# zerohd4869/MM-DFN

Measured on AMD Instinct MI355X. Metric: utterances/sec (fwd+bwd), IEMOCAP-shaped batch, higher is better.
Workload: dtype f32; 1 GPU; cfg2 (BASELINE configs[1]): B=16 dialogues/GPU, L=110, dims 100/100/512, 2 GCN layers, P=2, dropout 0.50; utterances_per_gpu=1760, parallelism=dp1

## Files before the change

### mm_dfn_amd/build.py

```python
import hashlib
import os
import shutil
import subprocess
import sys

HERE = os.path.dirname(os.path.abspath(__file__))
CSRC = os.path.join(HERE, "csrc")
LIBDIR = os.path.join(HERE, "lib")
LIBPATH = os.path.join(LIBDIR, "libmmdfn_hip.so")
TUNING_LIBPATH = os.path.join(LIBDIR, "libmmdfn_hip_tuning.so")
INCLUDE = os.path.join(os.path.dirname(HERE), "include")
ARCH = "gfx950"
NO_SPILL = {"gru.hip": ("gru_seq_bwd_kpart_kernelILi8ELi4ELi0ELi1E", "gru_seq_bwd_riders_kernelILb1E",
                        "gru_seq_fwd_io_kernelILi0ELi0ELi0ELi1E", "gru_seq_fwd_io_flags_kernelILi1E"),
            "lstm_seq.hip": ("lstm_seq_fwd_kernel", "lstm_seq_bwd_kernel"),
            "dialogue_rnn.hip": ("drnn_seq_fwd_kernel", "drnn_seq_bwd_kernel"),
            "cnn_features.hip": ("cnn_pool_fwd_kernel",)}


def sources():
    return sorted(os.path.join(CSRC, f) for f in os.listdir(CSRC) if f.endswith(".hip"))


def _digest():
    h = hashlib.sha256()
    files = sources() + sorted(os.path.join(CSRC, f) for f in os.listdir(CSRC) if f.endswith(".h"))
    files.append(os.path.join(INCLUDE, "mmdfn_hip.h"))
    for f in files:
        h.update(f.encode())
        with open(f, "rb") as fh:
            h.update(fh.read())
    return h.hexdigest()


def hipcc():
    exe = shutil.which("hipcc") or "/opt/rocm/bin/hipcc"
    if not os.path.exists(exe):
        raise RuntimeError("hipcc not found; libmmdfn_hip.so cannot be built")
    return exe


def build(force=False, verbose=True, tuning=False):
    import fcntl
    os.makedirs(LIBDIR, exist_ok=True)
    with open(os.path.join(LIBDIR, ".build.lock"), "w") as lock:
        fcntl.flock(lock, fcntl.LOCK_EX)
        try:
            return _build_locked(force, verbose, tuning)
        finally:
            fcntl.flock(lock, fcntl.LOCK_UN)


def _paths(tuning):
    lib = TUNING_LIBPATH if tuning else LIBPATH
    return lib, lib[:-3] + ".sha256", ("tuning_" if tuning else "")


def _build_locked(force, verbose, tuning):
    lib, stamp, prefix = _paths(tuning)
    digest = _digest()
    if not force and os.path.exists(lib) and os.path.exists(stamp):
        with open(stamp) as fh:
            if fh.read().strip() == digest:
                return lib
    objs = []
    jobs = []
    for src in sources():
        obj = os.path.join(LIBDIR, prefix + os.path.basename(src)[:-4] + ".o")
        cmd = [hipcc(), "--offload-arch=" + ARCH, "-O3", "-std=c++17", "-fPIC", "-I", INCLUDE, "-c", src, "-o", obj]
        if tuning:
            cmd.insert(1, "-DMMDFN_TUNING")
        if verbose:
            print(" ".join(cmd), flush=True)
        watch = NO_SPILL.get(os.path.basename(src))
        if watch:
            cmd.append("-Rpass-analysis=kernel-resource-usage")
            jobs.append((cmd, subprocess.Popen(cmd, stderr=subprocess.PIPE, text=True), watch))
        else:
            jobs.append((cmd, subprocess.Popen(cmd), None))
        objs.append(obj)
    for cmd, proc, watch in jobs:
        err = proc.communicate()[1] if watch else None
        if proc.wait() != 0:
            if err:
                sys.stderr.write(err)
            raise subprocess.CalledProcessError(proc.returncode, cmd)
        if watch:
            _check_no_spill(err, watch, cmd)
    cmd = [hipcc(), "--offload-arch=" + ARCH, "-shared", "-fPIC", "-o", lib] + objs
    if verbose:
        print(" ".join(cmd), flush=True)
    subprocess.check_call(cmd)
    with open(stamp, "w") as fh:
        fh.write(digest)
    return lib


def _check_no_spill(remarks, watch, cmd):
    name = None
    seen = set()
    for line in remarks.splitlines():
        if "Function Name:" in line:
            name = line.split("Function Name:")[1].split()[0]
        elif "ScratchSize [bytes/lane]:" in line and name and any(w in name for w in watch):
            seen.update(w for w in watch if w in name)
            if int(line.split("ScratchSize [bytes/lane]:")[1].split()[0]) != 0:
                raise RuntimeError("%s spills registers (%s): build.NO_SPILL lists it as a kernel that must run without "
                                   "scratch traffic" % (name, line.strip()))
    if len(seen) != len(watch):
        raise RuntimeError("no resource-usage remark for kernels matching %r (%s)" % (sorted(set(watch) - seen), " ".join(cmd)))


def is_stale(tuning=False):
    lib, stamp, _ = _paths(tuning)
    if not (os.path.exists(lib) and os.path.exists(stamp)):
        return True
    with open(stamp) as fh:
        return fh.read().strip() != _digest()


if __name__ == "__main__":
    print(build(force="--force" in sys.argv, tuning="--tuning" in sys.argv))
```

### mm_dfn_amd/csrc/gru.hip

```cpp
#include "mmdfn_internal.h"
#include "gemm_tn_split_body.h"
#include <type_traits>
#include <utility>
#include "keep_flags_body.h"
#include "../../include/mmdfn_hip.h"
#include <stdlib.h>

namespace {

constexpr int GH = 100;
constexpr int NT = 256;
constexpr int MAXG = 4;

constexpr int SCHED_MAX = 2048;
constexpr int MAXSEG = 16;

struct SegInfo {
    const int32_t* rank[MAXG];
    int P[MAXG];
    int BP[MAXG];
    int tdir[MAXG];
    int nslot;
    int slot_g[2 * MAXG];
    int slot_d[2 * MAXG];
// ... 1219 lines not shown
    };
    auto stash_block = [&](int buf) {
#pragma unroll
        for (int e = 0; e < NIN; ++e) {
            const int idx = tid + e * NTK;
            if (idx < TB * IN4) *reinterpret_cast<float4*>(&in_s[buf][0][0] + 4 * idx) = stage[e];
        }
    };
    auto flush_block = [&](int b) {
        for (int idx = tid; idx < TB * OUT4; idx += NTK) {
            const int sl = idx / OUT4;
            const int c4 = idx - sl * OUT4;
            const int sidx = b * TB + sl;
            if (sidx >= T) continue;
            int t;
            const int rw = step_row(sidx, t);
            const float4 v = *reinterpret_cast<const float4*>(&out_s[sl][4 * c4]);
            const int64_t o = ((int64_t)t * rows + rw) * (6 * GH) + dir * 3 * GH;
            if (c4 < 3 * GH / 4)
                *reinterpret_cast<float4*>(dgi + o + 4 * c4) = v;
            else
                __builtin_nontemporal_store(__builtin_bit_cast(f32x4, v), reinterpret_cast<f32x4*>(dgh + o + 4 * (c4 - 3 * GH / 4)));
        }
    };

    load_block(0);
    stash_block(0);
    if (nblocks > 1) load_block(1);
    __syncthreads();

    auto seg_end = [&](int prow) {
        if (dhinit != nullptr && ch.trunc) {
            f32x2 acc0 = {0.f, 0.f}, acc1 = {0.f, 0.f};
#pragma unroll
            for (int jj = 0; jj < JPW; ++jj) {
                const float dj = lane_bcast(dv[jj / 64], jj % 64);
                const f32x2 dd = {dj, dj};
                if (jj & 1) acc1 = __builtin_elementwise_fma(w[jj], dd, acc1);
                else acc0 = __builtin_elementwise_fma(w[jj], dd, acc0);
            }
            constexpr int PX = SEG ? 2 : 0;
            part[PX][wv][lane] = acc0[0] + acc1[0];
            part[PX][wv][lane + 64] = acc0[1] + acc1[1];
            __syncthreads();
#pragma unroll
            for (int q = 0; q < NGR; ++q) {
                float pr[NW];
#pragma unroll
                for (int w2 = 0; w2 < NW; ++w2) pr[w2] = part[PX][w2][uu[q]];
#pragma unroll
                for (int sp = 1; sp < NW; sp *= 2)
#pragma unroll
                    for (int w2 = 0; w2 + sp < NW; w2 += 2 * sp) pr[w2] += pr[w2 + sp];
                if (has[q] && gg[q] == 0) dhinit[(int64_t)prow * GH + uu[q]] = carry[q] + pr[0];
            }
        }
#pragma unroll
        for (int q = 0; q < NGR; ++q) {
            dv[q] = 0.f;
            carry[q] = 0.f;
        }
    };

    int step = 0;
    int seg_p = 0, bnd = 0x7fffffff;
    if constexpr (SEG) {
        int q = ch.nseg - 1;
        while (q >= 0 && seg_k[q] == 0) --q;
        int q2 = q - 1;
        while (q2 >= 0 && seg_k[q2] == 0) --q2;
        seg_p = __builtin_amdgcn_readfirstlane(q < 0 ? 0 : q);
        bnd = __builtin_amdgcn_readfirstlane(q2 >= 0 ? seg_k[q] : 0x7fffffff);
    }
    for (int b = 0; b < nblocks; ++b) {
        const int buf = b & 1;
        for (int sl = 0; sl < TB && step < T; ++sl, ++step) {
            const int pb = step & 1;
            if constexpr (SEG) {
                if (step == bnd) {
                    seg_end(row + seg_p);
                    int q = seg_p - 1;
                    while (q >= 0 && seg_k[q] == 0) --q;
                    seg_p = __builtin_amdgcn_readfirstlane(q);
                    int q2 = q - 1;
                    while (q2 >= 0 && seg_k[q2] == 0) --q2;
                    bnd = __builtin_amdgcn_readfirstlane(q2 >= 0 ? bnd + seg_k[q] : 0x7fffffff);
                }
            }
            const float* ip = &in_s[buf][sl][0];
            float iv[NGR][6];
#pragma unroll
            for (int q = 0; q < NGR; ++q)
#pragma unroll
                for (int e = 0; e < 6; ++e) iv[q][e] = ip[e * GH + uu[q]];
            f32x2 acc0 = {0.f, 0.f}, acc1 = {0.f, 0.f};
#pragma unroll
            for (int j4 = 0; j4 < JPW; j4 += GRP) {
                float dj[GRP];
#pragma unroll
                for (int e = 0; e < GRP; ++e) dj[e] = (j4 + e < JPW) ? lane_bcast(dv[(j4 + e) / 64], (j4 + e) % 64) : 0.f;
                if (GRP == 4) asm volatile("" : "+s"(dj[0]), "+s"(dj[GRP > 1 ? 1 : 0]), "+s"(dj[GRP > 2 ? 2 : 0]), "+s"(dj[GRP > 3 ? 3 : 0]));
#pragma unroll
                for (int e = 0; e < GRP; ++e) {
                    if (j4 + e >= JPW) continue;
                    const f32x2 dd = {dj[e], dj[e]};
                    if ((j4 + e) & 1) acc1 = __builtin_elementwise_fma(w[j4 + e], dd, acc1);
                    else acc0 = __builtin_elementwise_fma(w[j4 + e], dd, acc0);
                }
            }
            part[pb][wv][lane] = acc0[0] + acc1[0];
            part[pb][wv][lane + 64] = acc0[1] + acc1[1];
            __syncthreads();
            float* orow = &out_s[sl][0];
#pragma unroll
            for (int q = 0; q < NGR; ++q) {
                const int un = uu[q];
                float pr[NW];
#pragma unroll
                for (int w2 = 0; w2 < NW; ++w2) pr[w2] = part[pb][w2][un];
#pragma unroll
                for (int sp = 1; sp < NW; sp *= 2)
#pragma unroll
                    for (int w2 = 0; w2 + sp < NW; w2 += 2 * sp) pr[w2] += pr[w2 + sp];
                const float rec = pr[0];
                const float dh = iv[q][0] + carry[q] + rec;
                const float rr = iv[q][1], zz = iv[q][2], nn = iv[q][3], ghn = iv[q][4], hprev = iv[q][5];
                const float dn = dh * (1.0f - zz);
                const float dz = dh * (hprev - nn);
                carry[q] = dh * zz;
                const float dnpre = dn * (1.0f - nn * nn);
                const float drpre = dnpre * ghn * rr * (1.0f - rr);
                const float dzpre = dz * zz * (1.0f - zz);
                const float dghn = dnpre * rr;
                const float gi_v = gg[q] == 0 ? drpre : (gg[q] == 1 ? dzpre : dnpre);
                const float gh_v = gg[q] == 0 ? drpre : (gg[q] == 1 ? dzpre : dghn);
                if (has[q]) {
                    orow[jr[q]] = gi_v;
                    orow[3 * GH + jr[q]] = gh_v;
                }
                dv[q] = gh_v;
            }
        }
        __syncthreads();
        if (b + 1 < nblocks) stash_block(buf ^ 1);
        flush_block(b);
        if (b + 2 < nblocks) load_block(b + 2);
        __syncthreads();
    }
    if constexpr (SEG) {
        if (T > 0) seg_end(row + seg_p);
    }
}

constexpr int BWD_RING_D = 4;
constexpr int BWD_DIRECT_PART_B = 2 * 8 * PU * (int)sizeof(float);
constexpr int BWD_DIRECT_LDS = 84 * 1024;

static_assert(GH == 100, "the plane offsets of the direct body's requests are literals: 400 / 800 / 1200 bytes");
#define GRU_VM_LOAD(dst, off, base, lit) \
    asm volatile("global_load_dword %0, %1, %2" lit : "+v"(dst) : "v"(off), "s"(base))
template <int N>
__device__ __forceinline__ void vm_wait6(float (&r)[6]) {
    asm volatile("s_waitcnt vmcnt(%6)" : "+v"(r[0]), "+v"(r[1]), "+v"(r[2]), "+v"(r[3]), "+v"(r[4]), "+v"(r[5]) : "n"(N));
}

__device__ __forceinline__ void vm_store2(uint32_t off, float gi_v, float* pi, float gh_v, float* ph) {
    asm volatile("global_store_dword %0, %1, %2" : : "v"(off), "v"(gi_v), "s"(pi) : "memory");
    asm volatile("global_store_dword %0, %1, %2 nt" : : "v"(off), "v"(gh_v), "s"(ph) : "memory");
}
template <class F, int... K>
__device__ __forceinline__ void static_for(F& f, std::integer_sequence<int, K...>) {
    (f(std::integral_constant<int, K>{}), ...);
}
template <int J, int N, class F>
__device__ __forceinline__ void static_while(F& f, const int rem) {
    if constexpr (J < N) {
        if (J < rem) {
            f(std::integral_constant<int, J>{});
            static_while<J + 1, N>(f, rem);
        }
    }
}

__device__ __forceinline__ void gru_bwd_direct_body(const BwdGroups& G, const int bx, const int by, unsigned char* dyn) {
    constexpr int NW = 8, GRP = 4;
    constexpr int JPW = (3 * GH + NW - 1) / NW;
    constexpr int D = BWD_RING_D, NS = D + 1;
    static_assert(JPW <= 64, "a lane owns one gate row");
    static_assert(D >= 1 && D <= 7, "s_waitcnt vmcnt(8 D) must fit the 6-bit immediate");
    float (*part)[NW][PU] = reinterpret_cast<float (*)[NW][PU]>(dyn);

    int gidx = 0;
    while (gidx + 1 < G.n && bx >= G.slice0[gidx + 1]) ++gidx;
    const int dir = by;
    const int row = bx - G.slice0[gidx];
    const int T = G.T[gidx];
    const int rows = G.rows[gidx];
    if (T <= 0) return;
    const int tid = threadIdx.x, lane = tid & 63, wv = tid >> 6;
    const int j0 = JPW * wv;
    const float* __restrict__ dy = G.dy[gidx];
    const float* __restrict__ y = G.y[gidx];
    const float* __restrict__ gates = G.gates[gidx];
    const float* __restrict__ w_hh = G.w_hh[2 * gidx + dir];
    float* __restrict__ dgi = G.dgi[gidx];
    float* __restrict__ dgh = G.dgh[gidx];
    static_assert(3 * GH - (NW - 1) * JPW > 0, "every wave owns a gate row");

    const bool has1 = lane + 64 < GH;
    f32x2 w[JPW];
#pragma unroll
    for (int jj = 0; jj < JPW; ++jj) {
        const bool jok = j0 + jj < 3 * GH;
        const int jc = jok ? j0 + jj : 3 * GH - 1;
        w[jj][0] = jok ? w_hh[(int64_t)jc * GH + lane] : 0.f;
        w[jj][1] = (jok && has1) ? w_hh[(int64_t)jc * GH + lane + 64] : 0.f;
    }
#pragma unroll
    for (int jj = 0; jj < JPW; ++jj) pin_loaded(w[jj]);
    const bool has = lane < JPW && j0 + lane < 3 * GH;
    const int jr = has ? j0 + lane : 0;
    const int gg = jr / GH;
    const int uu = jr - gg * GH;
    uint32_t uoff = (uint32_t)uu * 4u, joff = (uint32_t)jr * 4u;
    float dv = 0.f, carry = 0.f;

    const int64_t dt = dir ? 1 : -1;
    const int64_t o0 = (int64_t)(dir ? 0 : T - 1) * rows + row;
    const int64_t st_y = dt * rows * (2 * GH), st_g = dt * rows * (8 * GH), st_o = dt * rows * (6 * GH);
    const float* pd = dy + o0 * (2 * GH) + dir * GH;
    const float* pg = gates + (o0 * 2 + dir) * (4 * GH);
    const float* py = y + o0 * (2 * GH) + dir * GH + (T > 1 ? st_y : 0);
    float* pi = dgi + o0 * (6 * GH) + dir * 3 * GH;
    float* ph = dgh + o0 * (6 * GH) + dir * 3 * GH;
    int f = 0;
    auto fetch = [&](float (&o6)[6]) {
        GRU_VM_LOAD(o6[0], uoff, pd, "");
        GRU_VM_LOAD(o6[1], uoff, pg, "");
        GRU_VM_LOAD(o6[2], uoff, pg, " offset:400");
        GRU_VM_LOAD(o6[3], uoff, pg, " offset:800");
        GRU_VM_LOAD(o6[4], uoff, pg, " offset:1200");
        GRU_VM_LOAD(o6[5], uoff, py, "");
        pd += (f + 1 < T) ? st_y : 0;
        pg += (f + 1 < T) ? st_g : 0;
        py += (f + 2 < T) ? st_y : 0;
        ++f;
    };

    float ring[NS][6];
#pragma unroll
    for (int k = 0; k < NS; ++k)
#pragma unroll
        for (int e = 0; e < 6; ++e) ring[k][e] = 0.f;
#pragma unroll
    for (int k = 0; k < D; ++k) fetch(ring[k]);

    auto run_step = [&](auto NC, const int step, float (&iv)[6]) {
        const int pb = step & 1;
        f32x2 acc0 = {0.f, 0.f}, acc1 = {0.f, 0.f};
#pragma unroll
        for (int j4 = 0; j4 < JPW; j4 += GRP) {
            float dj[GRP];
#pragma unroll
            for (int e = 0; e < GRP; ++e) dj[e] = (j4 + e < JPW) ? lane_bcast(dv, j4 + e) : 0.f;
            asm volatile("" : "+s"(dj[0]), "+s"(dj[1]), "+s"(dj[2]), "+s"(dj[3]));
#pragma unroll
            for (int e = 0; e < GRP; ++e) {
                if (j4 + e >= JPW) continue;
                const f32x2 dd = {dj[e], dj[e]};
                if ((j4 + e) & 1) acc1 = __builtin_elementwise_fma(w[j4 + e], dd, acc1);
                else acc0 = __builtin_elementwise_fma(w[j4 + e], dd, acc0);
            }
        }
        part[pb][wv][lane] = acc0[0] + acc1[0];
        part[pb][wv][lane + 64] = acc0[1] + acc1[1];
        __syncthreads();
        float pr[NW];
#pragma unroll
        for (int w2 = 0; w2 < NW; ++w2) pr[w2] = part[pb][w2][uu];
#pragma unroll
        for (int sp = 1; sp < NW; sp *= 2)
#pragma unroll
            for (int w2 = 0; w2 + sp < NW; w2 += 2 * sp) pr[w2] += pr[w2 + sp];
        const float rec = pr[0];
        vm_wait6<decltype(NC)::value>(iv);
        const float dh = iv[0] + carry + rec;
        const float rr = iv[1], zz = iv[2], nn = iv[3], ghn = iv[4];
        const float hprev = (step < T - 1) ? iv[5] : 0.f;
        const float dn = dh * (1.0f - zz);
        const float dz = dh * (hprev - nn);
        carry = dh * zz;
        float nn2 = nn * nn;
        asm("" : "+v"(nn2));
        const float dnpre = dn * (1.0f - nn2);
        const float drpre = dnpre * ghn * rr * (1.0f - rr);
        const float dzpre = dz * zz * (1.0f - zz);
        const float dghn = dnpre * rr;
        const float gi_v = gg == 0 ? drpre : (gg == 1 ? dzpre : dnpre);
        const float gh_v = gg == 0 ? drpre : (gg == 1 ? dzpre : dghn);
        dv = gh_v;
        asm volatile("" : "+v"(carry), "+v"(dv));
        if (has) {
            vm_store2(joff, gi_v, pi, gh_v, ph);
        }
        pi += st_o;
        ph += st_o;
    };

    const int T_trips = T - T % NS;
    for (int s0 = 0; s0 < T_trips; s0 += NS) {
        auto trip_step = [&](auto K) {
            constexpr int k = decltype(K)::value;
            fetch(ring[(k + D) % NS]);
            run_step(std::integral_constant<int, (6 * D + 2 * k < 8 * D ? 6 * D + 2 * k : 8 * D)>{}, s0 + k, ring[k]);
        };
        static_for(trip_step, std::make_integer_sequence<int, NS>{});
    }
    auto tail_step = [&](auto J) {
        constexpr int j = decltype(J)::value;
        run_step(std::integral_constant<int, 6 * (D - 1 - j) + 2 * j>{}, T_trips + j, ring[j]);
    };
    static_while<0, D>(tail_step, T - T_trips);
}

#ifndef MMDFN_FWD_RING_D
#define MMDFN_FWD_RING_D BWD_RING_D
#endif
#ifndef MMDFN_FWD_PAIR_STORES
#define MMDFN_FWD_PAIR_STORES 1
#endif
constexpr int FWD_RING_D = MMDFN_FWD_RING_D;
constexpr int FWD_PAIR_STORES = MMDFN_FWD_PAIR_STORES;
constexpr int FWD_DIRECT_LDS = BWD_DIRECT_LDS;

template <int N>
__device__ __forceinline__ void vm_wait3(float (&r)[3]) {
    asm volatile("s_waitcnt vmcnt(%3)" : "+v"(r[0]), "+v"(r[1]), "+v"(r[2]) : "n"(N));
}
#define GRU_VM_STORE(off, val, base, lit) \
    asm volatile("global_store_dword %0, %1, %2" lit : : "v"(off), "v"(val), "s"(base) : "memory")

__device__ __forceinline__ void gru_fwd_direct_body(const FwdGroups& G, const int bx, const int by) {
    constexpr int D = FWD_RING_D, NS = D + 1;
    constexpr int L = 3, S = FWD_PAIR_STORES ? 3 : 5;
    static_assert(D >= 1 && (L + S) * D <= 63, "s_waitcnt vmcnt((L + S) D) must fit the 6-bit immediate");
    __shared__ __attribute__((aligned(16))) float hs[2][GH + 4];

    int gidx = 0;
    while (gidx + 1 < G.n && bx >= G.slice0[gidx + 1]) ++gidx;
    const int dir = by;
    const int row = bx - G.slice0[gidx];
    const int T = G.T[gidx];
    const int rows = G.rows[gidx];
    if (T <= 0) return;
    const int tid = threadIdx.x;
    const int u = tid >> 1;
    const int half = tid & 1;
    const bool active = u < GH;
    const int uu = active ? u : GH - 1;
    const int kbase = half ? KH0 : 0;
    const int klen = half ? GH - KH0 : KH0;
    const float* __restrict__ gi = G.gi[gidx];
    const float* __restrict__ w_hh = G.w_hh[2 * gidx + dir];
    const float* __restrict__ b_hh = G.b_hh[2 * gidx + dir];
    float* __restrict__ y = G.y[gidx];
    float* __restrict__ gates = G.gates[gidx];
    f32x2 wr[KW / 2], wz[KW / 2], wn[KW / 2];
#pragma unroll
    for (int k = 0; k < KW; ++k) {
        const bool ok = k < klen;
        const int kk = kbase + (ok ? k : 0);
        wr[k >> 1][k & 1] = ok ? w_hh[(int64_t)(0 * GH + uu) * GH + kk] : 0.f;
        wz[k >> 1][k & 1] = ok ? w_hh[(int64_t)(1 * GH + uu) * GH + kk] : 0.f;
        wn[k >> 1][k & 1] = ok ? w_hh[(int64_t)(2 * GH + uu) * GH + kk] : 0.f;
    }
#pragma unroll
    for (int k = 0; k < KW / 2; ++k) {
        pin_loaded(wr[k]);
        pin_loaded(wz[k]);
        pin_loaded(wn[k]);
    }
    float bhr = b_hh[uu], bhz = b_hh[GH + uu], bhn = b_hh[2 * GH + uu];
    pin_loaded(bhr);
    pin_loaded(bhz);
    pin_loaded(bhn);
    const bool mine = active && half == 0;
    float hprev = 0.f;
    for (int i = tid; i < 2 * (GH + 4); i += NT) (&hs[0][0])[i] = 0.f;
    __syncthreads();

    const int64_t dt = dir ? -1 : 1;
    const int64_t o0 = (int64_t)(dir ? T - 1 : 0) * rows + row;
    const int64_t st_i = dt * rows * (6 * GH), st_y = dt * rows * (2 * GH), st_g = dt * rows * (8 * GH);
    const float* pi = gi + o0 * (6 * GH) + dir * 3 * GH;
    float* py = y + o0 * (2 * GH) + dir * GH;
    float* pg = gates + (o0 * 2 + dir) * (4 * GH);
    uint32_t ioff = (uint32_t)uu * 4u;
    uint32_t yoff = (uint32_t)uu * 4u;
    uint32_t goff = (uint32_t)uu * 4u + (FWD_PAIR_STORES && half ? 4u * GH : 0u);
    asm volatile("" : "+v"(ioff), "+v"(yoff), "+v"(goff));
    int f = 0;
    auto fetch = [&](float (&o3)[3]) {
        GRU_VM_LOAD(o3[0], ioff, pi, "");
        GRU_VM_LOAD(o3[1], ioff, pi, " offset:400");
        GRU_VM_LOAD(o3[2], ioff, pi, " offset:800");
        pi += (f + 1 < T) ? st_i : 0;
        ++f;
    };

    float ring[NS][3];
#pragma unroll
    for (int k = 0; k < NS; ++k)
#pragma unroll
        for (int e = 0; e < 3; ++e) ring[k][e] = 0.f;
#pragma unroll
    for (int k = 0; k < D; ++k) fetch(ring[k]);

    auto run_step = [&](auto NC, auto REQ, const int step, float (&iv)[3], float (&nx)[3]) {
        const int cur = step & 1;
        f32x2 ar0 = {0.f, 0.f}, az0 = {0.f, 0.f}, an0 = {0.f, 0.f}, ar1 = {0.f, 0.f}, az1 = {0.f, 0.f}, an1 = {0.f, 0.f};
        constexpr int HLOOK = 6;
        const uint32_t haddr = (uint32_t)(uintptr_t)((__attribute__((address_space(3))) const float*)(&hs[cur][kbase]));
        f32x4 hb[HLOOK];
#define GRU_LDS_RD(J)                                                                                        \
    asm volatile("ds_read_b128 %0, %1 offset:%2" : "=&v"(hb[(J) % HLOOK]) : "v"(haddr), "i"(16 * (J)) : "memory")
#define GRU_LDS_WAIT(N, J) asm volatile("s_waitcnt lgkmcnt(" #N ")" : "+v"(hb[(J) % HLOOK]) : : "memory")
#define GRU_GROUP(K4)                                                                                        \
    do {                                                                                                     \
        const f32x4 h4 = hb[(K4) % HLOOK];                                                                   \
        const f32x2 ha = {h4.x, h4.y}, hb2 = {h4.z, h4.w};                                                   \
        ar0 = __builtin_elementwise_fma(wr[2 * (K4)], ha, ar0);                                              \
        az0 = __builtin_elementwise_fma(wz[2 * (K4)], ha, az0);                                              \
        an0 = __builtin_elementwise_fma(wn[2 * (K4)], ha, an0);                                              \
        ar1 = __builtin_elementwise_fma(wr[2 * (K4) + 1], hb2, ar1);                                         \
        az1 = __builtin_elementwise_fma(wz[2 * (K4) + 1], hb2, az1);                                         \
        an1 = __builtin_elementwise_fma(wn[2 * (K4) + 1], hb2, an1);                                         \
    } while (0)
        GRU_LDS_RD(0); GRU_LDS_RD(1); GRU_LDS_RD(2); GRU_LDS_RD(3); GRU_LDS_RD(4); GRU_LDS_RD(5);
        if constexpr (decltype(REQ)::value) fetch(nx);
        GRU_LDS_WAIT(5, 0); GRU_GROUP(0); GRU_LDS_RD(6);
        GRU_LDS_WAIT(5, 1); GRU_GROUP(1); GRU_LDS_RD(7);
        GRU_LDS_WAIT(5, 2); GRU_GROUP(2); GRU_LDS_RD(8);
        GRU_LDS_WAIT(5, 3); GRU_GROUP(3); GRU_LDS_RD(9);
        GRU_LDS_WAIT(5, 4); GRU_GROUP(4); GRU_LDS_RD(10);
        GRU_LDS_WAIT(5, 5); GRU_GROUP(5); GRU_LDS_RD(11);
        GRU_LDS_WAIT(5, 6); GRU_GROUP(6); GRU_LDS_RD(12);
        GRU_LDS_WAIT(5, 7); GRU_GROUP(7);
        GRU_LDS_WAIT(4, 8); GRU_GROUP(8);
        GRU_LDS_WAIT(3, 9); GRU_GROUP(9);
        GRU_LDS_WAIT(2, 10); GRU_GROUP(10);
        GRU_LDS_WAIT(1, 11); GRU_GROUP(11);
        GRU_LDS_WAIT(0, 12); GRU_GROUP(12);
#undef GRU_GROUP
#undef GRU_LDS_WAIT
#undef GRU_LDS_RD
        float ar = (ar0.x + ar0.y) + (ar1.x + ar1.y);
        float az = (az0.x + az0.y) + (az1.x + az1.y);
        float an = (an0.x + an0.y) + (an1.x + an1.y);
        ar += pair_swap(ar);
        az += pair_swap(az);
        an += pair_swap(an);
        vm_wait3<decltype(NC)::value>(iv);
        const float g0 = iv[0], g1 = iv[1], g2 = iv[2];
        float ghn = an + bhn;
        float rr = sigmoidf_(g0 + ar + bhr);
        float zz = sigmoidf_(g1 + az + bhz);
        float nn = tanhf_(g2 + rr * ghn);
        float hnew = (1.0f - zz) * nn + zz * hprev;
        if (mine) hs[cur ^ 1][u] = hnew;
        asm volatile("" : "+v"(hnew), "+v"(rr), "+v"(zz), "+v"(nn), "+v"(ghn));
        hprev = hnew;
        if constexpr (FWD_PAIR_STORES) {
            const float va = half ? zz : rr, vb = half ? ghn : nn;
            if (active) {
                GRU_VM_STORE(goff, va, pg, " nt");
                GRU_VM_STORE(goff, vb, pg, " offset:800 nt");
                if (mine) GRU_VM_STORE(yoff, hnew, py, "");
            }
        } else {
            if (mine) {
                GRU_VM_STORE(yoff, hnew, py, "");
                GRU_VM_STORE(goff, rr, pg, " nt");
                GRU_VM_STORE(goff, zz, pg, " offset:400 nt");
                GRU_VM_STORE(goff, nn, pg, " offset:800 nt");
                GRU_VM_STORE(goff, ghn, pg, " offset:1200 nt");
            }
        }
        py += st_y;
        pg += st_g;
        __syncthreads();
    };

    const int T_trips = T - T % NS;
    const std::true_type yes{};
    const std::false_type no{};
    if (T_trips > 0) {
        auto first_step = [&](auto K) {
            constexpr int k = decltype(K)::value;
            run_step(std::integral_constant<int, L * D + S * k>{}, yes, k, ring[k], ring[(k + D) % NS]);
        };
        static_for(first_step, std::make_integer_sequence<int, NS>{});
        for (int s0 = NS; s0 < T_trips; s0 += NS) {
            auto trip_step = [&](auto K) {
                constexpr int k = decltype(K)::value;
                run_step(std::integral_constant<int, (L + S) * D>{}, yes, s0 + k, ring[k], ring[(k + D) % NS]);
            };
            static_for(trip_step, std::make_integer_sequence<int, NS>{});
        }
    }
    auto tail_step = [&](auto J) {
        constexpr int j = decltype(J)::value;
        run_step(std::integral_constant<int, L * (D - 1 - j) + S * j>{}, no, T_trips + j, ring[j], ring[j]);
    };
    static_while<0, D>(tail_step, T - T_trips);
}

template <int NW, int GRP, int SEG, int DIRECT = 0>
__global__ __launch_bounds__(64 * NW) void gru_seq_bwd_kpart_kernel(BwdGroups G) {
    if constexpr (DIRECT) {
        static_assert(NW == 8 && GRP == 4 && SEG == 0, "the direct body is the plain eight-wave recurrence");
        extern __shared__ __attribute__((aligned(16))) unsigned char direct_smem[];
        gru_bwd_direct_body(G, (int)blockIdx.x, (int)blockIdx.y, direct_smem);
    } else {
        gru_bwd_kpart_body<NW, GRP, SEG, false>(G, (int)blockIdx.x, (int)blockIdx.y, nullptr);
    }
}


template <bool DIRECT>
__global__ __launch_bounds__(512) void gru_seq_bwd_riders_kernel(const BwdGroups G, const TnRiderSegs rq, const int nslots,
                                                                 const int ngru8) {
    extern __shared__ __attribute__((aligned(16))) unsigned char rider_smem[];
    const int bid = (int)blockIdx.x;
    if (bid < 2 * nslots) {
        if constexpr (DIRECT) gru_bwd_direct_body(G, bid % nslots, bid / nslots, rider_smem);
        else gru_bwd_kpart_body<8, 4, 0, true>(G, bid % nslots, bid / nslots, rider_smem);
    } else if (bid >= ngru8) {
        tnsb::tns_block<0>(rq, bid - ngru8, rider_smem, nullptr);
    }
}

__global__ __launch_bounds__(1024) void gru_tab_reduce_kernel(const float* __restrict__ dy, const int32_t* __restrict__ kout,
                                                              const float* __restrict__ dhinit, float* __restrict__ dyt,
                                                              int rows, int T, int dir) {
    constexpr int C4 = GH / 4;
    constexpr int RG = 32;
    __shared__ float4 red[RG][32];
    const int t = blockIdx.x;
    const int c4 = threadIdx.x & 31, rg = threadIdx.x >> 5;
    const int cc = c4 < C4 ? c4 : C4 - 1;
    float4 acc = make_float4(0.f, 0.f, 0.f, 0.f);
    for (int r0 = rg; r0 < rows; r0 += 8 * RG) {
        float4 v[8], h[8];
        float m[8], mh[8];
#pragma unroll
        for (int e = 0; e < 8; ++e) {
            const int r = r0 + e * RG;
            const int rc = r < rows ? r : rows - 1;
            const int k = kout[rc];
            m[e] = (r < rows && k <= t) ? 1.f : 0.f;
            mh[e] = (r < rows && k == t && k >= 1) ? 1.f : 0.f;
            v[e] = *reinterpret_cast<const float4*>(dy + ((int64_t)t * rows + rc) * (2 * GH) + dir * GH + 4 * cc);
            h[e] = *reinterpret_cast<const float4*>(dhinit + (int64_t)rc * GH + 4 * cc);
        }
#pragma unroll
        for (int e = 0; e < 8; ++e) {
            if (m[e] != 0.f) { acc.x += v[e].x; acc.y += v[e].y; acc.z += v[e].z; acc.w += v[e].w; }
            if (mh[e] != 0.f) { acc.x += h[e].x; acc.y += h[e].y; acc.z += h[e].z; acc.w += h[e].w; }
        }
    }
    red[rg][c4] = acc;
    __syncthreads();
    if (rg == 0 && c4 < C4) {
        float4 a = red[0][c4];
#pragma unroll
        for (int g = 1; g < RG; ++g) {
            const float4 v = red[g][c4];
            a.x += v.x; a.y += v.y; a.z += v.z; a.w += v.w;
        }
        *reinterpret_cast<float4*>(dyt + (int64_t)t * (2 * GH) + dir * GH + 4 * c4) = a;
        *reinterpret_cast<float4*>(dyt + (int64_t)t * (2 * GH) + (1 - dir) * GH + 4 * c4) = make_float4(0.f, 0.f, 0.f, 0.f);
    }
}

int seg_slots(SegInfo& S, int ngroups, const int* rows, const int* T, const int32_t* const* rank, const int* P, const int* BP,
              const int* tdir) {
    for (int g = 0; g < ngroups; ++g) {
        S.rank[g] = rank ? rank[g] : nullptr;
        S.P[g] = 1; S.BP[g] = 1; S.tdir[g] = -1;
        if (S.rank[g] != nullptr) {
            if (P[g] <= 0 || P[g] > MAXSEG || BP[g] <= 0 || BP[g] % P[g] || rows[g] % BP[g] || T[g] >= 4096 ||
                (int64_t)P[g] * T[g] > SCHED_MAX || tdir[g] < -1 || tdir[g] > 1) return -1;
            S.P[g] = P[g]; S.BP[g] = BP[g]; S.tdir[g] = tdir[g];
        } else if (T[g] > SCHED_MAX) {
            return -1;
        }
    }
    int ns = 0, start = 0;
    for (int pass = 0; pass < 2; ++pass)
        for (int g = 0; g < ngroups; ++g)
            for (int d = 0; d < 2; ++d) {
                const bool trunc = S.rank[g] != nullptr && S.tdir[g] == d;
                if ((int)trunc != pass) continue;
                S.slot_g[ns] = g; S.slot_d[ns] = d; S.slot_start[ns] = start;
                start += trunc ? rows[g] / S.P[g] : rows[g];
                ++ns;
            }
    S.nslot = ns;
    S.slot_start[ns] = start;
    return start;
}

int mfma_min_chains() {
#ifdef MMDFN_TUNING
    if (const char* e = getenv("MMDFN_GRU_MFMA_MIN")) return atoi(e);
#endif
    return 1024;
}

bool kpart_any_size() {
#ifdef MMDFN_TUNING
    const char* e = getenv("MMDFN_GRU_KPART_BWD");
    return e != nullptr && e[0] == '2';
#else
    return false;
#endif
}

bool use_kpart_bwd() {
#ifdef MMDFN_TUNING
    const char* e = getenv("MMDFN_GRU_KPART_BWD");
    if (e != nullptr) return e[0] != '0';
#endif
    return true;
}

bool use_staged_bwd() {
#ifdef MMDFN_TUNING
    const char* e = getenv("MMDFN_GRU_BWD_STAGED");
    if (e != nullptr) return e[0] == '1';
#endif
    return false;
}

bool use_staged_fwd() {
#ifdef MMDFN_TUNING
    const char* e = getenv("MMDFN_GRU_FWD_STAGED");
    if (e != nullptr) return e[0] == '1';
#endif
    return false;
}

static_assert(BWD_DIRECT_PART_B <= BWD_DIRECT_LDS && BWD_DIRECT_PART_B <= tnsb::LDS_B, "the partial sums sit in the launch's LDS");
static_assert(2 * BWD_DIRECT_LDS > 160 * 1024, "one recurrence workgroup per CU");
static_assert(2 * FWD_DIRECT_LDS > 160 * 1024, "one forward recurrence workgroup per CU");

int pick_r(int ngroups, const int* rows) {
#ifdef MMDFN_TUNING
    if (const char* e = getenv("MMDFN_GRU_R")) {
        const int v = atoi(e);
        if (v == 1 || v == 2 || v == 4) return v;
    }
#endif
    for (int R : {1, 2, 4}) {
        int wg = 0;
        for (int g = 0; g < ngroups; ++g) wg += (rows[g] + R - 1) / R;
        if (2 * wg <= 4096) return R;
    }
    return 4;
}

}

GruForm mmdfn_gru_form(int ngroups, const int* rows) {
    GruForm f = {false, 1, 0, 0};
    if (ngroups <= 0 || ngroups > MAXG) return f;
    int chains = 0;
    for (int g = 0; g < ngroups; ++g) {
        if (rows[g] <= 0) return f;
        chains += 2 * rows[g];
    }
    f.R = pick_r(ngroups, rows);
    f.mfma = chains > mfma_min_chains();
    const int per_wg = f.mfma ? 16 : f.R;
    for (int g = 0; g < ngroups; ++g) f.slices += (rows[g] + per_wg - 1) / per_wg;
    if ((f.mfma || f.R == 1) && 2 * f.slices < MMDFN_CUS) f.idle_cus = MMDFN_CUS - 2 * f.slices;
    return f;
}

extern "C" int mmdfn_gru_seq_fwd(int ngroups, const float* const* gi, const float* const* w_hh,
                                 const float* const* b_hh, float* const* y, float* const* gates, const int* rows,
                                 const int* T, int H, void* riders, void* stream) {
    if (ngroups <= 0 || ngroups > MAXG || H != GH) return -1;
    const GruForm f = mmdfn_gru_form(ngroups, rows);
    const int R = f.R;
    FwdGroups G;
    if (!mmdfn_gru_fill_fwd(G, ngroups, gi, w_hh, b_hh, y, gates, rows, T, R)) return -1;
#ifdef MMDFN_TUNING
    if (const char* e = getenv("MMDFN_GRU_ABL")) G.abl = atoi(e);
#endif
    const int sl = G.slice0[ngroups];
    dim3 grid(sl, 2), block(NT);
    hipStream_t s = (hipStream_t)stream;
    MmdfnRiders* rd = (MmdfnRiders*)riders;
    if (f.mfma && G.abl == 0) return mmdfn_launch_gru_fwd_mfma(f, ngroups, gi, w_hh, b_hh, y, gates, rows, T, rd, s);
    bool io_wave = (R == 1) && (2 * sl <= MMDFN_CUS);
#ifdef MMDFN_TUNING
    if (const char* e = getenv("MMDFN_GRU_IO")) io_wave = io_wave && e[0] != '0';
#endif
    bool scalar_fma = false;
#ifdef MMDFN_TUNING
    if (const char* e = getenv("MMDFN_GRU_SCALAR_FMA")) scalar_fma = e[0] == '1';
#endif
#ifdef MMDFN_TUNING
#define GRU_IO_ABL(A) if (io_wave && G.abl == A) { hipLaunchKernelGGL((gru_seq_fwd_io_kernel<0, A, 0>), grid, dim3(320), 0, s, G); MMDFN_CHECK_LAUNCH(); return 0; }
    GRU_IO_ABL(1) GRU_IO_ABL(2) GRU_IO_ABL(4) GRU_IO_ABL(8) GRU_IO_ABL(16) GRU_IO_ABL(3) GRU_IO_ABL(11) GRU_IO_ABL(31) GRU_IO_ABL(23) GRU_IO_ABL(64)
#undef GRU_IO_ABL
#endif
    if (io_wave && !scalar_fma && f.idle_cus > 0 && rd != nullptr && rd->flag_job_valid) {
        const kfb::FlagJob J = rd->flag_job;
        rd->flag_job_valid = false;
#ifdef MMDFN_TUNING
        if (use_staged_fwd()) {
            int64_t nr5 = (J.n8 + 319) / 320;
            if (nr5 > f.idle_cus) nr5 = f.idle_cus;
            hipLaunchKernelGGL(gru_seq_fwd_io_flags_kernel<0>, dim3(2 * sl + (int)nr5), dim3(320), 0, s, G, J, sl);
            MMDFN_CHECK_LAUNCH();
            return 0;
        }
#endif
        int64_t nr = (J.n8 + NT - 1) / NT;
        if (nr > f.idle_cus) nr = f.idle_cus;
        if (int e = mmdfn_allow_big_lds(gru_seq_fwd_io_flags_kernel<1>)) return e;
        hipLaunchKernelGGL(gru_seq_fwd_io_flags_kernel<1>, dim3(2 * sl + (int)nr), dim3(NT), FWD_DIRECT_LDS, s, G, J, sl);
        MMDFN_CHECK_LAUNCH();
        return 0;
    }
    if (io_wave && scalar_fma) hipLaunchKernelGGL((gru_seq_fwd_io_kernel<1, 0, 0>), grid, dim3(320), 0, s, G);
#ifdef MMDFN_TUNING
    else if (io_wave && use_staged_fwd()) hipLaunchKernelGGL((gru_seq_fwd_io_kernel<0, 0, 0>), grid, dim3(320), 0, s, G);
#endif
    else if (io_wave) {
        if (int e = mmdfn_allow_big_lds(gru_seq_fwd_io_kernel<0, 0, 0, 1>)) return e;
        hipLaunchKernelGGL((gru_seq_fwd_io_kernel<0, 0, 0, 1>), grid, dim3(NT), FWD_DIRECT_LDS, s, G);
    }
    else if (R == 1) hipLaunchKernelGGL((gru_seq_fwd_kernel<1, 0>), grid, block, 0, s, G);
    else if (R == 2) hipLaunchKernelGGL((gru_seq_fwd_kernel<2, 0>), grid, block, 0, s, G);
    else hipLaunchKernelGGL((gru_seq_fwd_kernel<4, 0>), grid, block, 0, s, G);
    MMDFN_CHECK_LAUNCH();
    return 0;
}

extern "C" int mmdfn_gru_seq_bwd(int ngroups, const float* const* dy, const float* const* y,
                                 const float* const* gates, const float* const* w_hh, float* const* dgi,
                                 float* const* dgh, const int* rows, const int* T, int H, void* riders, void* stream) {
    if (ngroups <= 0 || ngroups > MAXG || H != GH) return -1;
    const GruForm f = mmdfn_gru_form(ngroups, rows);
    const int R = f.R;
    BwdGroups G;
    if (!mmdfn_gru_fill_bwd(G, ngroups, dy, y, gates, w_hh, dgi, dgh, rows, T, R)) return -1;
    const int sl = G.slice0[ngroups];
    dim3 grid(sl, 2), block(NT);
    hipStream_t s = (hipStream_t)stream;
    MmdfnRiders* rd = (MmdfnRiders*)riders;
    if (f.mfma) return mmdfn_launch_gru_bwd_mfma(f, ngroups, dy, y, gates, w_hh, dgi, dgh, rows, T, rd, s);
    if (R == 1 && (2 * sl <= MMDFN_CUS || kpart_any_size()) && use_kpart_bwd()) {
        if (f.idle_cus > 0 && rd != nullptr && rd->rider.valid && rd->rider.tq.n <= MMDFN_RIDER_MAXSEG) {
            const TnSplitSegs& rp = rd->rider.tq;
            TnRiderSegs rq;
            mmdfn_seg_copy(rq, rp);
            const int ngru8 = (2 * sl + 7) & ~7;
            const dim3 rgrid(ngru8 + rp.wg_prefix[rp.n]);
#ifdef MMDFN_TUNING
            if (use_staged_bwd()) {
                if (int e = mmdfn_allow_big_lds(gru_seq_bwd_riders_kernel<false>)) return e;
                hipLaunchKernelGGL(gru_seq_bwd_riders_kernel<false>, rgrid, dim3(512), tnsb::LDS_B, s, G, rq, sl, ngru8);
                MMDFN_CHECK_LAUNCH();
                return mmdfn_riders_launched(rd, s);
            }
#endif
            if (int e = mmdfn_allow_big_lds(gru_seq_bwd_riders_kernel<true>)) return e;
            hipLaunchKernelGGL(gru_seq_bwd_riders_kernel<true>, rgrid, dim3(512), tnsb::LDS_B, s, G, rq, sl, ngru8);
            MMDFN_CHECK_LAUNCH();
            return mmdfn_riders_launched(rd, s);
        }
#ifdef MMDFN_TUNING
        if (use_staged_bwd()) {
            hipLaunchKernelGGL((gru_seq_bwd_kpart_kernel<8, 4, 0>), grid, dim3(512), 0, s, G);
            MMDFN_CHECK_LAUNCH();
            return 0;
        }
#endif
        if (int e = mmdfn_allow_big_lds(gru_seq_bwd_kpart_kernel<8, 4, 0, 1>)) return e;
        hipLaunchKernelGGL((gru_seq_bwd_kpart_kernel<8, 4, 0, 1>), grid, dim3(512), BWD_DIRECT_LDS, s, G);
    }
    else if (R == 1) hipLaunchKernelGGL((gru_seq_bwd_kernel<1, 0>), grid, block, 0, s, G);
    else if (R == 2) hipLaunchKernelGGL((gru_seq_bwd_kernel<2, 0>), grid, block, 0, s, G);
    else hipLaunchKernelGGL((gru_seq_bwd_kernel<4, 0>), grid, block, 0, s, G);
    MMDFN_CHECK_LAUNCH();
    return 0;
}

extern "C" int mmdfn_gru_seq_bwd_idle_cus(int ngroups, const int* rows) {
    const GruForm f = mmdfn_gru_form(ngroups, rows);
    return (f.mfma || use_kpart_bwd()) ? f.idle_cus : 0;
}

extern "C" int mmdfn_gru_seq_fwd_takes_flags(int ngroups, const int* rows) {
    return mmdfn_gru_form(ngroups, rows).idle_cus > 0 ? 1 : 0;
}

extern "C" int mmdfn_gru_seq_bwd_step_ns(int ngroups, const int* rows) {
    return mmdfn_gru_form(ngroups, rows).mfma ? 2300 : 650;
}

extern "C" int mmdfn_gru_seq_fwd_seg(int ngroups, const float* const* gi, const float* const* w_hh,
                                     const float* const* b_hh, float* const* y, float* const* gates, const int* rows,
                                     const int* T, int H, const int32_t* const* rank, const int* P, const int* BP,
                                     const int* tdir, const float* const* ytab, void* stream) {
    if (ngroups <= 0 || ngroups > MAXG || H != GH) return -1;
    FwdGroups G;
    if (!mmdfn_gru_fill_fwd(G, ngroups, gi, w_hh, b_hh, y, gates, rows, T, 0)) return -1;
    for (int g = 0; g < ngroups; ++g) {
        G.ytab[g] = ytab ? ytab[g] : nullptr;
        if (G.ytab[g] != nullptr && (rank == nullptr || rank[g] == nullptr || tdir[g] != 1)) return -1;
    }
    const int nchains = seg_slots(G.seg, ngroups, rows, T, rank, P, BP, tdir);
    if (nchains <= 0) return -1;
    bool io_wave = nchains <= MMDFN_CUS;
#ifdef MMDFN_TUNING
    if (const char* e = getenv("MMDFN_GRU_IO")) io_wave = e[0] != '0';
#endif
#ifdef MMDFN_TUNING
    if (const char* e = getenv("MMDFN_GRU_ABL")) {
        const int a = atoi(e);
#define GRU_SEG_ABL(A) if (io_wave && a == A) { hipLaunchKernelGGL((gru_seq_fwd_io_kernel<0, A, 1>), dim3(nchains), dim3(320), 0, (hipStream_t)stream, G); MMDFN_CHECK_LAUNCH(); return 0; }
        GRU_SEG_ABL(32)
#undef GRU_SEG_ABL
    }
#endif
    if (io_wave) hipLaunchKernelGGL((gru_seq_fwd_io_kernel<0, 0, 1>), dim3(nchains), dim3(320), 0, (hipStream_t)stream, G);
    else hipLaunchKernelGGL((gru_seq_fwd_kernel<1, 1>), dim3(nchains), dim3(NT), 0, (hipStream_t)stream, G);
    MMDFN_CHECK_LAUNCH();
    return 0;
}

extern "C" int mmdfn_gru_seq_bwd_seg(int ngroups, const float* const* dy, const float* const* y,
                                     const float* const* gates, const float* const* w_hh, float* const* dgi,
                                     float* const* dgh, const int* rows, const int* T, int H,
                                     const int32_t* const* rank, const int* P, const int* BP, const int* tdir,
                                     float* const* dhinit, int32_t* const* kout, void* stream) {
    if (ngroups <= 0 || ngroups > MAXG || H != GH) return -1;
    BwdGroups G;
    if (!mmdfn_gru_fill_bwd(G, ngroups, dy, y, gates, w_hh, dgi, dgh, rows, T, 0)) return -1;
    for (int g = 0; g < ngroups; ++g) {
        G.dhinit[g] = dhinit ? dhinit[g] : nullptr;
        G.kout[g] = kout ? kout[g] : nullptr;
        if ((G.dhinit[g] != nullptr) != (G.kout[g] != nullptr)) return -1;
        if (G.dhinit[g] != nullptr && (rank == nullptr || rank[g] == nullptr || tdir[g] != 1)) return -1;
    }
    const int nchains = seg_slots(G.seg, ngroups, rows, T, rank, P, BP, tdir);
    if (nchains <= 0) return -1;
    bool kpart = nchains <= MMDFN_CUS;
#ifdef MMDFN_TUNING
    if (const char* e = getenv("MMDFN_GRU_KPART_BWD")) kpart = e[0] != '0';
#endif
    if (kpart) hipLaunchKernelGGL((gru_seq_bwd_kpart_kernel<8, 4, 1>), dim3(nchains), dim3(512), 0, (hipStream_t)stream, G);
    else hipLaunchKernelGGL((gru_seq_bwd_kernel<1, 1>), dim3(nchains), dim3(NT), 0, (hipStream_t)stream, G);
    MMDFN_CHECK_LAUNCH();
    return 0;
}

extern "C" int mmdfn_gru_tab_reduce(const float* dy, const int32_t* kout, const float* dhinit, float* dyt, int rows, int T,
                                    int H, int dir, void* stream) {
    if (H != GH || rows <= 0 || T <= 0 || dir < 0 || dir > 1) return -1;
    hipLaunchKernelGGL(gru_tab_reduce_kernel, dim3(T), dim3(1024), 0, (hipStream_t)stream, dy, kout, dhinit, dyt, rows, T, dir);
    MMDFN_CHECK_LAUNCH();
    return 0;
}
```

Baseline: 2.390 million utterances/s.

## Restructure GRU backward recurrence into lane-group form with DPP reductions

The direct GRU backward recurrence body gains a lane-group form as the new default. In it, each 16-lane group holds weights for a 4-unit block, reads the previous step's dgh from a small double-buffered LDS image, and reduces partial sums with DPP moves. This replaces the per-row lane broadcasts and the cross-wave LDS partial-sum reduction used by the old wave-partition form. The cost is an extra LDS write per step plus a block barrier after every step. The old wave-partition form and a no-broadcast probe variant stay available behind tuning env flags, and the advertised per-step cost for the scheduler is lowered.

New measurement: 2.372 million utterances/s, median of 2. Within noise of the previous version (-0.8%).

```diff
diff --git a/mm_dfn_amd/build.py b/mm_dfn_amd/build.py
--- a/mm_dfn_amd/build.py
+++ b/mm_dfn_amd/build.py
@@ -11,7 +11,7 @@
 TUNING_LIBPATH = os.path.join(LIBDIR, "libmmdfn_hip_tuning.so")
 INCLUDE = os.path.join(os.path.dirname(HERE), "include")
 ARCH = "gfx950"
-NO_SPILL = {"gru.hip": ("gru_seq_bwd_kpart_kernelILi8ELi4ELi0ELi1E", "gru_seq_bwd_riders_kernelILb1E",
+NO_SPILL = {"gru.hip": ("gru_seq_bwd_kpart_kernelILi8ELi4ELi0ELi1E", "gru_seq_bwd_riders_kernelILi1E",
                         "gru_seq_fwd_io_kernelILi0ELi0ELi0ELi1E", "gru_seq_fwd_io_flags_kernelILi1E"),
             "lstm_seq.hip": ("lstm_seq_fwd_kernel", "lstm_seq_bwd_kernel"),
             "dialogue_rnn.hip": ("drnn_seq_fwd_kernel", "drnn_seq_bwd_kernel"),
diff --git a/mm_dfn_amd/csrc/gru.hip b/mm_dfn_amd/csrc/gru.hip
--- a/mm_dfn_amd/csrc/gru.hip
+++ b/mm_dfn_amd/csrc/gru.hip
@@ -1395,7 +1395,13 @@
     }
 }
 
-constexpr int BWD_RING_D = 4;
+#ifndef MMDFN_BWD_RING_D
+#define MMDFN_BWD_RING_D 4
+#endif
+constexpr int BWD_RING_D = MMDFN_BWD_RING_D;
+constexpr int BWD_LANEGROUP = 1, BWD_WAVEPART = 2, BWD_WAVEPART_NOBCAST = 3;
+constexpr int BWD_LG_NI = 19, BWD_LG_CH = 20, BWD_LG_IMG = 16 * BWD_LG_CH;
+constexpr int BWD_LG_IMG_B = 2 * BWD_LG_IMG * (int)sizeof(float);
 constexpr int BWD_DIRECT_PART_B = 2 * 8 * PU * (int)sizeof(float);
 constexpr int BWD_DIRECT_LDS = 84 * 1024;
 
@@ -1425,13 +1431,19 @@
     }
 }
 
+template <int FORM>
 __device__ __forceinline__ void gru_bwd_direct_body(const BwdGroups& G, const int bx, const int by, unsigned char* dyn) {
     constexpr int NW = 8, GRP = 4;
     constexpr int JPW = (3 * GH + NW - 1) / NW;
     constexpr int D = BWD_RING_D, NS = D + 1;
+    constexpr bool LG = FORM == BWD_LANEGROUP;
+    static_assert(FORM == BWD_LANEGROUP || FORM == BWD_WAVEPART || FORM == BWD_WAVEPART_NOBCAST, "a form of the direct body");
     static_assert(JPW <= 64, "a lane owns one gate row");
+    static_assert(JPW == 2 * BWD_LG_NI && BWD_LG_NI < BWD_LG_CH && BWD_LG_CH % 4 == 0 && GH % 4 == 0 && GH / 4 <= 4 * NW,
+                  "lane-group form: chains of 19 rows in images of 20 floats, 25 blocks of 4 units on 32 DPP rows");
     static_assert(D >= 1 && D <= 7, "s_waitcnt vmcnt(8 D) must fit the 6-bit immediate");
     float (*part)[NW][PU] = reinterpret_cast<float (*)[NW][PU]>(dyn);
+    float* img = reinterpret_cast<float*>(dyn);
 
     int gidx = 0;
     while (gidx + 1 < G.n && bx >= G.slice0[gidx + 1]) ++gidx;
@@ -1450,23 +1462,59 @@
     float* __restrict__ dgh = G.dgh[gidx];
     static_assert(3 * GH - (NW - 1) * JPW > 0, "every wave owns a gate row");
 
-    const bool has1 = lane + 64 < GH;
+    const int l16 = lane & 15;
+    const int blk = 8 * (lane >> 4) + wv;
+    const bool bok = blk < GH / 4;
+    const int u0 = bok ? 4 * blk : 0;
     f32x2 w[JPW];
-#pragma unroll
-    for (int jj = 0; jj < JPW; ++jj) {
-        const bool jok = j0 + jj < 3 * GH;
-        const int jc = jok ? j0 + jj : 3 * GH - 1;
-        w[jj][0] = jok ? w_hh[(int64_t)jc * GH + lane] : 0.f;
-        w[jj][1] = (jok && has1) ? w_hh[(int64_t)jc * GH + lane + 64] : 0.f;
+    if constexpr (LG) {
+        const int jb = JPW * (l16 >> 1) + (l16 & 1);
+#pragma unroll
+        for (int i = 0; i < BWD_LG_NI; ++i) {
+            const int j = jb + 2 * i;
+            const float* __restrict__ wr = w_hh + (int64_t)(j < 3 * GH ? j : 3 * GH - 1) * GH + u0;
+            w[2 * i][0] = wr[0];
+            w[2 * i][1] = wr[1];
+            w[2 * i + 1][0] = wr[2];
+            w[2 * i + 1][1] = wr[3];
+        }
+#pragma unroll
+        for (int jj = 0; jj < JPW; ++jj) pin_loaded(w[jj]);
+#pragma unroll
+        for (int i = 0; i < BWD_LG_NI; ++i) {
+            const bool jok = bok && jb + 2 * i < 3 * GH;
+            const f32x2 zero = {0.f, 0.f};
+            w[2 * i] = jok ? w[2 * i] : zero;
+            w[2 * i + 1] = jok ? w[2 * i + 1] : zero;
+        }
+    } else {
+        const bool has1 = lane + 64 < GH;
+#pragma unroll
+        for (int jj = 0; jj < JPW; ++jj) {
+            const bool jok = j0 + jj < 3 * GH;
+            const int jc = jok ? j0 + jj : 3 * GH - 1;
+            w[jj][0] = jok ? w_hh[(int64_t)jc * GH + lane] : 0.f;
+            w[jj][1] = (jok && has1) ? w_hh[(int64_t)jc * GH + lane + 64] : 0.f;
+        }
     }
 #pragma unroll
     for (int jj = 0; jj < JPW; ++jj) pin_loaded(w[jj]);
-    const bool has = lane < JPW && j0 + lane < 3 * GH;
-    const int jr = has ? j0 + lane : 0;
+    const int ku = (l16 & 3) ^ ((l16 & 4) ? 3 : 0);
+    const bool has = LG ? (bok && l16 < 12) : (lane < JPW && j0 + lane < 3 * GH);
+    const int jr = !has ? 0 : (LG ? (l16 >> 2) * GH + u0 + ku : j0 + lane);
     const int gg = jr / GH;
     const int uu = jr - gg * GH;
+    const int woff = (2 * (jr / JPW) + ((jr % JPW) & 1)) * BWD_LG_CH + ((jr % JPW) >> 1);
+    if constexpr (LG) {
+        static_assert(2 * BWD_LG_IMG <= 2 * 64 * NW, "two stores per thread clear the images");
+        img[tid] = 0.f;
+        if (tid < 2 * BWD_LG_IMG - 64 * NW) img[64 * NW + tid] = 0.f;
+        __syncthreads();
+    }
     uint32_t uoff = (uint32_t)uu * 4u, joff = (uint32_t)jr * 4u;
     float dv = 0.f, carry = 0.f;
+    float nobcast = 0.f;
+    if constexpr (FORM == BWD_WAVEPART_NOBCAST) nobcast = lane_bcast(__int_as_float(T), 0);
 
     const int64_t dt = dir ? 1 : -1;
     const int64_t o0 = (int64_t)(dir ? 0 : T - 1) * rows + row;
@@ -1500,32 +1548,59 @@
 
     auto run_step = [&](auto NC, const int step, float (&iv)[6]) {
         const int pb = step & 1;
-        f32x2 acc0 = {0.f, 0.f}, acc1 = {0.f, 0.f};
-#pragma unroll
-        for (int j4 = 0; j4 < JPW; j4 += GRP) {
-            float dj[GRP];
-#pragma unroll
-            for (int e = 0; e < GRP; ++e) dj[e] = (j4 + e < JPW) ? lane_bcast(dv, j4 + e) : 0.f;
-            asm volatile("" : "+s"(dj[0]), "+s"(dj[1]), "+s"(dj[2]), "+s"(dj[3]));
-#pragma unroll
-            for (int e = 0; e < GRP; ++e) {
-                if (j4 + e >= JPW) continue;
-                const f32x2 dd = {dj[e], dj[e]};
-                if ((j4 + e) & 1) acc1 = __builtin_elementwise_fma(w[j4 + e], dd, acc1);
-                else acc0 = __builtin_elementwise_fma(w[j4 + e], dd, acc0);
-            }
-        }
-        part[pb][wv][lane] = acc0[0] + acc1[0];
-        part[pb][wv][lane + 64] = acc0[1] + acc1[1];
-        __syncthreads();
-        float pr[NW];
-#pragma unroll
-        for (int w2 = 0; w2 < NW; ++w2) pr[w2] = part[pb][w2][uu];
-#pragma unroll
-        for (int sp = 1; sp < NW; sp *= 2)
-#pragma unroll
-            for (int w2 = 0; w2 + sp < NW; w2 += 2 * sp) pr[w2] += pr[w2 + sp];
-        const float rec = pr[0];
+        float rec;
+        if constexpr (LG) {
+            const float* rp = img + pb * BWD_LG_IMG + l16 * BWD_LG_CH;
+            f32x4 d4[BWD_LG_CH / 4];
+#pragma unroll
+            for (int q = 0; q < BWD_LG_CH / 4; ++q) d4[q] = *reinterpret_cast<const f32x4*>(rp + 4 * q);
+            f32x2 a01 = {0.f, 0.f}, a23 = {0.f, 0.f};
+#pragma unroll
+            for (int i = 0; i < BWD_LG_NI; ++i) {
+                const f32x2 dd = {d4[i / 4][i % 4], d4[i / 4][i % 4]};
+                a01 = __builtin_elementwise_fma(w[2 * i], dd, a01);
+                a23 = __builtin_elementwise_fma(w[2 * i + 1], dd, a23);
+            }
+            float s4[4] = {a01[0], a01[1], a23[0], a23[1]};
+#pragma unroll
+            for (int e = 0; e < 4; ++e) s4[e] += mmdfn_dpp_mov<0xB1>(s4[e]);
+#pragma unroll
+            for (int e = 0; e < 4; ++e) s4[e] += mmdfn_dpp_mov<0x4E>(s4[e]);
+            const float lo = (ku & 1) ? s4[1] : s4[0], hi = (ku & 1) ? s4[3] : s4[2];
+            rec = (ku & 2) ? hi : lo;
+            rec += mmdfn_dpp_mov<0x141>(rec);
+            rec += mmdfn_dpp_mov<0x140>(rec);
+        } else {
+            f32x2 acc0 = {0.f, 0.f}, acc1 = {0.f, 0.f};
+#pragma unroll
+            for (int j4 = 0; j4 < JPW; j4 += GRP) {
+                float dj[GRP];
+#pragma unroll
+                for (int e = 0; e < GRP; ++e) {
+                    if constexpr (FORM == BWD_WAVEPART_NOBCAST) dj[e] = nobcast;
+                    else dj[e] = (j4 + e < JPW) ? lane_bcast(dv, j4 + e) : 0.f;
+                }
+                asm volatile("" : "+s"(dj[0]), "+s"(dj[1]), "+s"(dj[2]), "+s"(dj[3]));
+#pragma unroll
+                for (int e = 0; e < GRP; ++e) {
+                    if (j4 + e >= JPW) continue;
+                    const f32x2 dd = {dj[e], dj[e]};
+                    if ((j4 + e) & 1) acc1 = __builtin_elementwise_fma(w[j4 + e], dd, acc1);
+                    else acc0 = __builtin_elementwise_fma(w[j4 + e], dd, acc0);
+                }
+            }
+            part[pb][wv][lane] = acc0[0] + acc1[0];
+            part[pb][wv][lane + 64] = acc0[1] + acc1[1];
+            __syncthreads();
+            float pr[NW];
+#pragma unroll
+            for (int w2 = 0; w2 < NW; ++w2) pr[w2] = part[pb][w2][uu];
+#pragma unroll
+            for (int sp = 1; sp < NW; sp *= 2)
+#pragma unroll
+                for (int w2 = 0; w2 + sp < NW; w2 += 2 * sp) pr[w2] += pr[w2 + sp];
+            rec = pr[0];
+        }
         vm_wait6<decltype(NC)::value>(iv);
         const float dh = iv[0] + carry + rec;
         const float rr = iv[1], zz = iv[2], nn = iv[3], ghn = iv[4];
@@ -1545,9 +1620,11 @@
         asm volatile("" : "+v"(carry), "+v"(dv));
         if (has) {
             vm_store2(joff, gi_v, pi, gh_v, ph);
+            if constexpr (LG) img[(pb ^ 1) * BWD_LG_IMG + woff] = gh_v;
         }
         pi += st_o;
         ph += st_o;
+        if constexpr (LG) __syncthreads();
     };
 
     const int T_trips = T - T % NS;
@@ -1763,20 +1840,20 @@
     if constexpr (DIRECT) {
         static_assert(NW == 8 && GRP == 4 && SEG == 0, "the direct body is the plain eight-wave recurrence");
         extern __shared__ __attribute__((aligned(16))) unsigned char direct_smem[];
-        gru_bwd_direct_body(G, (int)blockIdx.x, (int)blockIdx.y, direct_smem);
+        gru_bwd_direct_body<DIRECT>(G, (int)blockIdx.x, (int)blockIdx.y, direct_smem);
     } else {
         gru_bwd_kpart_body<NW, GRP, SEG, false>(G, (int)blockIdx.x, (int)blockIdx.y, nullptr);
     }
 }
 
 
-template <bool DIRECT>
+template <int DIRECT>
 __global__ __launch_bounds__(512) void gru_seq_bwd_riders_kernel(const BwdGroups G, const TnRiderSegs rq, const int nslots,
                                                                  const int ngru8) {
     extern __shared__ __attribute__((aligned(16))) unsigned char rider_smem[];
     const int bid = (int)blockIdx.x;
     if (bid < 2 * nslots) {
-        if constexpr (DIRECT) gru_bwd_direct_body(G, bid % nslots, bid / nslots, rider_smem);
+        if constexpr (DIRECT) gru_bwd_direct_body<DIRECT>(G, bid % nslots, bid / nslots, rider_smem);
         else gru_bwd_kpart_body<8, 4, 0, true>(G, bid % nslots, bid / nslots, rider_smem);
     } else if (bid >= ngru8) {
         tnsb::tns_block<0>(rq, bid - ngru8, rider_smem, nullptr);
@@ -1886,6 +1963,14 @@
     return false;
 }
 
+int wavepart_bwd() {
+#ifdef MMDFN_TUNING
+    const char* e = getenv("MMDFN_GRU_BWD_WAVEPART");
+    if (e != nullptr && (e[0] == '1' || e[0] == '2')) return e[0] - '0';
+#endif
+    return 0;
+}
+
 bool use_staged_fwd() {
 #ifdef MMDFN_TUNING
     const char* e = getenv("MMDFN_GRU_FWD_STAGED");
@@ -1895,6 +1980,7 @@
 }
 
 static_assert(BWD_DIRECT_PART_B <= BWD_DIRECT_LDS && BWD_DIRECT_PART_B <= tnsb::LDS_B, "the partial sums sit in the launch's LDS");
+static_assert(BWD_LG_IMG_B <= BWD_DIRECT_LDS && BWD_LG_IMG_B <= tnsb::LDS_B, "the dgh images sit in the launch's LDS");
 static_assert(2 * BWD_DIRECT_LDS > 160 * 1024, "one recurrence workgroup per CU");
 static_assert(2 * FWD_DIRECT_LDS > 160 * 1024, "one forward recurrence workgroup per CU");
 
@@ -2016,14 +2102,20 @@
             const dim3 rgrid(ngru8 + rp.wg_prefix[rp.n]);
 #ifdef MMDFN_TUNING
             if (use_staged_bwd()) {
-                if (int e = mmdfn_allow_big_lds(gru_seq_bwd_riders_kernel<false>)) return e;
-                hipLaunchKernelGGL(gru_seq_bwd_riders_kernel<false>, rgrid, dim3(512), tnsb::LDS_B, s, G, rq, sl, ngru8);
+                if (int e = mmdfn_allow_big_lds(gru_seq_bwd_riders_kernel<0>)) return e;
+                hipLaunchKernelGGL(gru_seq_bwd_riders_kernel<0>, rgrid, dim3(512), tnsb::LDS_B, s, G, rq, sl, ngru8);
                 MMDFN_CHECK_LAUNCH();
                 return mmdfn_riders_launched(rd, s);
             }
+            if (wavepart_bwd()) {
+                if (int e = mmdfn_allow_big_lds(gru_seq_bwd_riders_kernel<BWD_WAVEPART>)) return e;
+                hipLaunchKernelGGL(gru_seq_bwd_riders_kernel<BWD_WAVEPART>, rgrid, dim3(512), tnsb::LDS_B, s, G, rq, sl, ngru8);
+                MMDFN_CHECK_LAUNCH();
+                return mmdfn_riders_launched(rd, s);
+            }
 #endif
-            if (int e = mmdfn_allow_big_lds(gru_seq_bwd_riders_kernel<true>)) return e;
-            hipLaunchKernelGGL(gru_seq_bwd_riders_kernel<true>, rgrid, dim3(512), tnsb::LDS_B, s, G, rq, sl, ngru8);
+            if (int e = mmdfn_allow_big_lds(gru_seq_bwd_riders_kernel<BWD_LANEGROUP>)) return e;
+            hipLaunchKernelGGL(gru_seq_bwd_riders_kernel<BWD_LANEGROUP>, rgrid, dim3(512), tnsb::LDS_B, s, G, rq, sl, ngru8);
             MMDFN_CHECK_LAUNCH();
             return mmdfn_riders_launched(rd, s);
         }
@@ -2033,6 +2125,18 @@
             MMDFN_CHECK_LAUNCH();
             return 0;
         }
+        if (wavepart_bwd() == 1) {
+            if (int e = mmdfn_allow_big_lds(gru_seq_bwd_kpart_kernel<8, 4, 0, BWD_WAVEPART>)) return e;
+            hipLaunchKernelGGL((gru_seq_bwd_kpart_kernel<8, 4, 0, BWD_WAVEPART>), grid, dim3(512), BWD_DIRECT_LDS, s, G);
+            MMDFN_CHECK_LAUNCH();
+            return 0;
+        }
+        if (wavepart_bwd() == 2) {
+            if (int e = mmdfn_allow_big_lds(gru_seq_bwd_kpart_kernel<8, 4, 0, BWD_WAVEPART_NOBCAST>)) return e;
+            hipLaunchKernelGGL((gru_seq_bwd_kpart_kernel<8, 4, 0, BWD_WAVEPART_NOBCAST>), grid, dim3(512), BWD_DIRECT_LDS, s, G);
+            MMDFN_CHECK_LAUNCH();
+            return 0;
+        }
 #endif
         if (int e = mmdfn_allow_big_lds(gru_seq_bwd_kpart_kernel<8, 4, 0, 1>)) return e;
         hipLaunchKernelGGL((gru_seq_bwd_kpart_kernel<8, 4, 0, 1>), grid, dim3(512), BWD_DIRECT_LDS, s, G);
@@ -2054,7 +2158,7 @@
 }
 
 extern "C" int mmdfn_gru_seq_bwd_step_ns(int ngroups, const int* rows) {
-    return mmdfn_gru_form(ngroups, rows).mfma ? 2300 : 650;
+    return mmdfn_gru_form(ngroups, rows).mfma ? 2300 : 580;
 }
 
 extern "C" int mmdfn_gru_seq_fwd_seg(int ngroups, const float* const* gi, const float* const* w_hh,
```
